# krea-ai/realtime-video

Hardware: AMD Instinct MI355X
Metric: frames/sec at 832x480, 4-step 14B T2V (per-step DiT latency in config) (higher is better)
Workload: dtype bf16

## Files before the change

### realtime_video_amd/csrc/vae_conv.hip

```cpp
#include "gemm_core.h"
#include "rtv_internal.h"

namespace rtv {

struct ConvParams {
  const uint16_t* in;
  const uint16_t* w;
  uint16_t* out;
  const uint16_t* bias;
  const uint16_t* residual;
  const uint16_t* zeros;
  int out_ld, res_ld;
  int T, H, W;
  int inH, inW;
  int Cin, Cout;
  int kt, kh, kw;
  int w_taps;
  int ups;
  int sy, st;
  int pad_h, pad_w;
  int limH, limW;
  int y_out0, y_in0;
  int in_rows;
  int gather;
// ... 513 lines not shown
    const int n = n0 + c * 8;
    u32x4 tv = *(const u32x4*)(img + conv_img_off<TN>(row, c, 0));
    if (y >= p.H || x >= p.W) continue;
    const size_t m = ((size_t)t * p.H + y) * p.W + x;
    if (p.residual) {
      const u32x4 rr = res_pre[ps];
#pragma unroll
      for (int i = 0; i < 4; ++i) {
        float a0, a1, r0, r1;
        unpack_f16x2(tv[i], a0, a1);
        unpack_f16x2(rr[i], r0, r1);
        tv[i] = pack_f16x2(a0 + r0, a1 + r1);
      }
    }
    *(u32x4*)(p.out + m * p.out_ld + n) = tv;
  }
}

namespace ch4 {
using namespace ch;
constexpr int THREADS4 = 256;
constexpr int HP = 10, WP = 5;
constexpr int A_ACC = 0, A_FRAG = 192, FRAG_SET = 28;
template <int ACC, int WF, int AF>
__device__ __forceinline__ void mfma_aaa() {
  asm volatile("v_mfma_f32_32x32x16_f16 a[%c0:%c1], a[%c2:%c3], a[%c4:%c5], a[%c0:%c1]" ::"n"(ACC), "n"(ACC + 15), "n"(WF), "n"(WF + 3),
               "n"(AF), "n"(AF + 3));
}
template <int DST, int OFF>
__device__ __forceinline__ void lds_read128_a(uint32_t lds_addr) {
  asm volatile("ds_read_b128 a[%c1:%c2], %0 offset:%3" ::"v"(lds_addr), "n"(DST), "n"(DST + 3), "n"(OFF));
}
template <int DST>
__device__ __forceinline__ void acc_zero() {
  asm volatile("v_accvgpr_write_b32 a[%c0], 0" ::"n"(DST));
}
template <int SRC>
__device__ __forceinline__ float acc_read() {
  float r;
  asm volatile("v_accvgpr_read_b32 %0, a[%c1]" : "=v"(r) : "n"(SRC));
  return r;
}
#define RTV_CH4_ACC \
  "a0", "a15", "a31", "a47", "a63", "a79", "a95", "a111", "a127", "a143", "a159", "a175", "a191", "a207", "a223", "a239", "a247"
}

template <int LAB>
__global__ __launch_bounds__(ch4::THREADS4, 1) void conv_halo4_kernel(ConvParams p, int tiles_x, int tiles_y) {
  using namespace ch4;
  extern __shared__ __attribute__((aligned(16))) char smem[];
  const int tid = threadIdx.x;
  const int lane = tid & 63;
  const int wave = __builtin_amdgcn_readfirstlane(tid >> 6);
  const int l31 = lane & 31, gl = lane >> 5;

  const int tiles_n = p.Cout / 96;
  const int id = xcd_remap(blockIdx.x, p.T * tiles_y * tiles_x * tiles_n);
  const int tn = id % tiles_n;
  int rest = id / tiles_n;
  const int tx = rest % tiles_x;
  rest /= tiles_x;
  const int ty = rest % tiles_y, t = rest / tiles_y;
  const int x0 = tx * TW, y0 = ty * TH, n0 = tn * 96;

  const int cpk = p.Cin / 32;
  const int G = p.kt * cpk;
  const int slice = p.inH * p.inW * p.Cin;
  const int taps = p.w_taps;

  uint32_t h_voff[HP], h_lds[HP];
#pragma unroll
  for (int i = 0; i < HP; ++i) {
    const int piece = min(wave * HP + i, HREAL - 1);
    h_lds[i] = piece * 1024;
    const int q = piece * 16 + (lane >> 2);
    const int hr = q / HPITCH, hc = q - hr * HPITCH;
    const int y = y0 - 1 + hr, x = x0 - 1 + hc;
    const int yi = p.y_out0 + y;
    const bool ok = q < HPIX && yi >= 0 && yi < p.limH && x >= 0 && x < p.limW;
    const int ys = p.ups ? (yi >> 1) - p.y_in0 : y, xs = p.ups ? x >> 1 : x;
    const int c = (lane & 3) ^ ((hc >> 2) & 3);
    h_voff[i] = ok ? (uint32_t)(((t * p.inH + ys) * p.inW + xs) * p.Cin + c * 8) * 2u : 0x80000000u;
  }
  uint32_t w_voff[WP], w_lds[WP];
#pragma unroll
  for (int i = 0; i < WP; ++i) {
    int piece = wave * WP + i;
    if (piece >= WREAL) piece -= 2;
    w_lds[i] = piece * 1024;
    const int dx = piece / 6, f = (piece % 6) * 16 + (lane >> 2);
    const int c = (lane & 3) ^ ((f >> 2) & 3);
    w_voff[i] = (uint32_t)(((n0 + f) * taps + dx) * p.Cin + c * 8) * 2u;
  }
  const __amdgpu_buffer_rsrc_t rsrcI = __builtin_amdgcn_make_buffer_rsrc((void*)p.in, 0, 0x80000000, 0x00020000);
  const __amdgpu_buffer_rsrc_t rsrcW = __builtin_amdgcn_make_buffer_rsrc((void*)p.w, 0, 0x7fffffff, 0x00020000);
  const uint32_t lds0 = (uint32_t)(uintptr_t)(RTV_LDS const char*)smem;
  auto issue_h = [&](uint32_t soff, uint32_t buf, auto ic) __attribute__((always_inline)) {
    constexpr int I = decltype(ic)::value;
    RTV_LDS void* dst = (RTV_LDS void*)(uintptr_t)(lds0 + buf * (uint32_t)HBYTES + h_lds[I]);
    __builtin_amdgcn_raw_ptr_buffer_load_lds(rsrcI, dst, 16, h_voff[I], soff, 0, 0);
  };
  auto issue_w = [&](uint32_t soff, auto slotc, auto ic) __attribute__((always_inline)) {
    constexpr int I = decltype(ic)::value, SLOT = decltype(slotc)::value;
    RTV_LDS void* dst = (RTV_LDS void*)(uintptr_t)(lds0 + (uint32_t)(2 * HBYTES + SLOT * WROW_BYTES) + w_lds[I]);
    __builtin_amdgcn_raw_ptr_buffer_load_lds(rsrcW, dst, 16, w_voff[I], soff, 0, 0);
  };
  auto h_soff = [&](int dt, int cb) __attribute__((always_inline)) { return (uint32_t)(dt * slice + cb * 32) * 2u; };
  auto w_soff = [&](int dt, int cb, int dy) __attribute__((always_inline)) {
    return (uint32_t)((dt * 9 + dy * 3) * p.Cin + cb * 32) * 2u;
  };

  uint32_t a_base[3][2], b_addr[3][2];
#pragma unroll
  for (int ks = 0; ks < 2; ++ks) {
#pragma unroll
    for (int dx = 0; dx < 3; ++dx) {
      const int hc = l31 + dx;
      a_base[dx][ks] = lds0 + (uint32_t)(((4 * wave) * HPITCH + hc) * 64 + (((2 * ks + gl) ^ ((hc >> 2) & 3)) << 4));
    }
#pragma unroll
    for (int dy = 0; dy < 3; ++dy)
      b_addr[dy][ks] = lds0 + (uint32_t)(2 * HBYTES + dy * WROW_BYTES + l31 * 64 + (((2 * ks + gl) ^ ((l31 >> 2) & 3)) << 4));
  }
  uint32_t a_cur[3][2], a_nxt[3][2];
  auto frag_read = [&](auto dyc, auto cic, auto setc, auto nc, const uint32_t (&aa)[3][2]) __attribute__((always_inline)) {
    constexpr int DY = decltype(dyc)::value, CI = decltype(cic)::value, SET = decltype(setc)::value, N = decltype(nc)::value;
    constexpr int dx = CI >> 1, ks = CI & 1;
    if constexpr (N < 3) lds_read128_a<A_FRAG + FRAG_SET * SET + 4 * N, dx * (96 * 64) + N * (32 * 64)>(b_addr[DY][ks]);
    else lds_read128_a<A_FRAG + FRAG_SET * SET + 12 + 4 * (N - 3), ((N - 3) + DY) * (HPITCH * 64)>(aa[dx][ks]);
  };

  asm volatile("" ::: RTV_CH4_ACC);
  sfor<0, 192>([&](auto ic) __attribute__((always_inline)) { acc_zero<A_ACC + decltype(ic)::value>(); });

  sfor<0, HP>([&](auto ic) __attribute__((always_inline)) { issue_h(h_soff(0, 0), 0u, ic); });
  sfor<0, WP>([&](auto ic) __attribute__((always_inline)) { issue_w(w_soff(0, 0, 0), IC<0>{}, ic); });
  sfor<0, WP>([&](auto ic) __attribute__((always_inline)) { issue_w(w_soff(0, 0, 1), IC<1>{}, ic); });
  asm volatile("s_waitcnt vmcnt(5)" ::: "memory");
  __builtin_amdgcn_s_barrier();
#pragma unroll
  for (int ks = 0; ks < 2; ++ks)
#pragma unroll
    for (int dx = 0; dx < 3; ++dx) a_cur[dx][ks] = a_base[dx][ks];
  sfor<0, 7>([&](auto nc) __attribute__((always_inline)) { frag_read(IC<0>{}, IC<0>{}, IC<0>{}, nc, a_cur); });

  int dt = 0, cb = 0;
  for (int g = 0; g < G; ++g) {
    const uint32_t nsel = (g & 1) ? 0u : (uint32_t)HBYTES;
    const bool more = g + 1 < G;
    const int cb1 = cb + 1 == cpk ? 0 : cb + 1, dt1 = cb + 1 == cpk ? dt + 1 : dt;
    uint32_t ws[3], hs;
    ws[0] = w_soff(dt, cb, 2);
    ws[1] = more ? w_soff(dt1, cb1, 0) : ws[0];
    ws[2] = more ? w_soff(dt1, cb1, 1) : ws[0];
    hs = more ? h_soff(dt1, cb1) : h_soff(dt, cb);
    const uint32_t nbuf = (uint32_t)((g + 1) & 1);
#pragma unroll
    for (int ks = 0; ks < 2; ++ks)
#pragma unroll
      for (int dx = 0; dx < 3; ++dx) a_nxt[dx][ks] = a_base[dx][ks] + nsel;
    sfor<0, 3>([&](auto dyc) __attribute__((always_inline)) {
      constexpr int DY = decltype(dyc)::value;
      sfor<0, 6>([&](auto cic) __attribute__((always_inline)) {
        constexpr int CI = decltype(cic)::value, SET = CI & 1;
        asm volatile("s_waitcnt lgkmcnt(0)");
        sfor<0, 12>([&](auto nc) __attribute__((always_inline)) {
          constexpr int n = decltype(nc)::value, mi = n / 3, ni = n % 3;
          mfma_aaa<A_ACC + (mi * 3 + ni) * 16, A_FRAG + FRAG_SET * SET + 4 * ni, A_FRAG + FRAG_SET * SET + 12 + 4 * mi>();
          __builtin_amdgcn_sched_barrier(0);
          if constexpr (CI < 5) {
            if constexpr (n < 7) frag_read(dyc, IC<CI + 1>{}, IC<SET ^ 1>{}, nc, a_cur);
            if constexpr (LAB != 1) {
              if constexpr (CI == 0 && n >= 7) issue_w(ws[DY], IC<(DY + 2) % 3>{}, IC<n - 7>{});
              if constexpr (DY == 0 && (CI == 1 || CI == 2) && n >= 7) issue_h(hs, nbuf, IC<(CI - 1) * 5 + n - 7>{});
            }
          } else {
            if constexpr (n == 2) {
              if constexpr (LAB == 1) asm volatile("s_waitcnt vmcnt(0)" ::: "memory");
              else if constexpr (DY == 2) asm volatile("s_waitcnt vmcnt(5)" ::: "memory");
              else asm volatile("s_waitcnt vmcnt(15)" ::: "memory");
              __builtin_amdgcn_s_barrier();
              __builtin_amdgcn_sched_barrier(0);
            }
            if constexpr (n >= 3 && n < 10) {
              if constexpr (DY < 2) frag_read(IC<DY + 1>{}, IC<0>{}, IC<SET ^ 1>{}, IC<n - 3>{}, a_cur);
              else frag_read(IC<0>{}, IC<0>{}, IC<SET ^ 1>{}, IC<n - 3>{}, a_nxt);
            }
          }
          __builtin_amdgcn_sched_barrier(0);
        });
      });
    });
#pragma unroll
    for (int ks = 0; ks < 2; ++ks)
#pragma unroll
      for (int dx = 0; dx < 3; ++dx) a_cur[dx][ks] = a_nxt[dx][ks];
    dt = dt1;
    cb = cb1;
  }
  asm volatile("s_waitcnt lgkmcnt(0)");
  asm volatile("s_waitcnt vmcnt(0)" ::: "memory");
  __builtin_amdgcn_s_barrier();
  asm volatile("s_nop 15\n\ts_nop 7");
  if constexpr (LAB == 2) {
    if (acc_read<0>() == 12345.678f) p.out[tid] = 1;
    return;
  }

  constexpr int TM = 4, TN = 3, CPR = TN * 4;
  u32x4 res_pre[TM * 32 * CPR / 64];
  if (p.residual) {
#pragma unroll
    for (int ps = 0; ps < TM * 32 * CPR / 64; ++ps) {
      const int q = ps * 64 + lane;
      const int row = q / CPR, c = q - row * CPR;
      const int y = y0 + 4 * wave + (row >> 5), x = x0 + (row & 31);
      res_pre[ps] = u32x4{0u, 0u, 0u, 0u};
      if (y < p.H && x < p.W) res_pre[ps] = *(const u32x4*)(p.residual + (((size_t)t * p.H + y) * p.W + x) * p.res_ld + n0 + c * 8);
    }
  }
  char* img = smem + wave * (TM * 32 * TN * 64);
  sfor<0, TM>([&](auto mic) __attribute__((always_inline)) {
    constexpr int mi = decltype(mic)::value;
    f32x16 accv[TN];
    sfor<0, TN * 16>([&](auto ic) __attribute__((always_inline)) {
      constexpr int i = decltype(ic)::value;
      accv[i >> 4][i & 15] = acc_read<A_ACC + mi * 48 + i>();
    });
    const int row = mi * 32 + l31;
    float yv[TN][4][4];
    float ssq = 0.f;
#pragma unroll
    for (int ni = 0; ni < TN; ++ni)
#pragma unroll
      for (int rq = 0; rq < 4; ++rq) {
        const int n = n0 + ni * 32 + rq * 8 + gl * 4;
        float v[4] = {accv[ni][rq * 4 + 0], accv[ni][rq * 4 + 1], accv[ni][rq * 4 + 2], accv[ni][rq * 4 + 3]};
        if (p.bias) {
          const u32x2 bb = *(const u32x2*)(p.bias + n);
          v[0] += f16_to_f32(bb[0] & 0xffff);
          v[1] += f16_to_f32(bb[0] >> 16);
          v[2] += f16_to_f32(bb[1] & 0xffff);
          v[3] += f16_to_f32(bb[1] >> 16);
        }
        u32x2 o;
        o[0] = pack_f16x2(v[0], v[1]);
        o[1] = pack_f16x2(v[2], v[3]);
        if (p.norm_gamma) {
          unpack_f16x2(o[0], yv[ni][rq][0], yv[ni][rq][1]);
          unpack_f16x2(o[1], yv[ni][rq][2], yv[ni][rq][3]);
#pragma unroll
          for (int i = 0; i < 4; ++i) ssq += yv[ni][rq][i] * yv[ni][rq][i];
        } else {
          *(u32x2*)(img + conv_img_off<TN>(row, ni * 4 + rq, gl)) = o;
        }
      }
    if (p.norm_gamma) {
      ssq += __shfl_xor(ssq, 32, 64);
      const float inv = sqrtf(96.f) / fmaxf(sqrtf(ssq), 1e-12f);
#pragma unroll
      for (int ni = 0; ni < TN; ++ni)
#pragma unroll
        for (int rq = 0; rq < 4; ++rq) {
          const u32x2 gg = *(const u32x2*)(p.norm_gamma + ni * 32 + rq * 8 + gl * 4);
          float g4[4];
          unpack_f16x2(gg[0], g4[0], g4[1]);
          unpack_f16x2(gg[1], g4[2], g4[3]);
          float z[4];
#pragma unroll
          for (int i = 0; i < 4; ++i) z[i] = silu(yv[ni][rq][i] * inv * g4[i]);
          u32x2 o;
          o[0] = pack_f16x2(z[0], z[1]);
          o[1] = pack_f16x2(z[2], z[3]);
          *(u32x2*)(img + conv_img_off<TN>(row, ni * 4 + rq, gl)) = o;
        }
    }
  });
  asm volatile("s_waitcnt lgkmcnt(0)" ::: "memory");
  __builtin_amdgcn_sched_barrier(0);
  constexpr int PASSES = TM * 32 * CPR / 64;
#pragma unroll
  for (int ps = 0; ps < PASSES; ++ps) {
    const int q = ps * 64 + lane;
    const int row = q / CPR, c = q - row * CPR;
    const int y = y0 + 4 * wave + (row >> 5), x = x0 + (row & 31);
    const int n = n0 + c * 8;
    u32x4 tv = *(const u32x4*)(img + conv_img_off<TN>(row, c, 0));
    if (y >= p.H || x >= p.W) continue;
    const size_t m = ((size_t)t * p.H + y) * p.W + x;
    if (p.residual) {
      const u32x4 rr = res_pre[ps];
#pragma unroll
      for (int i = 0; i < 4; ++i) {
        float a0, a1, r0, r1;
        unpack_f16x2(tv[i], a0, a1);
        unpack_f16x2(rr[i], r0, r1);
        tv[i] = pack_f16x2(a0 + r0, a1 + r1);
      }
    }
    *(u32x4*)(p.out + m * p.out_ld + n) = tv;
  }
}

__global__ __attribute__((amdgpu_flat_work_group_size(256, 256), amdgpu_waves_per_eu(1, 2))) void conv_halo4p_kernel(ConvParams p, int tiles_x,
                                                                                                                      int tiles_y) {
  using namespace ch4;
  constexpr int A_ACC = 8, A_FRAG = 200;
  extern __shared__ __attribute__((aligned(16))) char smem[];
  const int tid = threadIdx.x;
  const int lane = tid & 63;
  const int wave = __builtin_amdgcn_readfirstlane(tid >> 6);
  const int l31 = lane & 31, gl = lane >> 5;

  const int tiles_n = p.Cout / 96;
  const int total = p.T * tiles_y * tiles_x * tiles_n;
  const int stride = gridDim.x;
  const int cpk = p.Cin / 32;
  const int G = p.kt * cpk;
  const int slice = p.inH * p.inW * p.Cin;
  const int taps = p.w_taps;

  auto decode = [&](int vid, int& t, int& y0, int& x0, int& n0) __attribute__((always_inline)) {
    const int id = xcd_remap(vid, total);
    const int tn = id % tiles_n;
    int rest = id / tiles_n;
    const int tx = rest % tiles_x;
    rest /= tiles_x;
    const int ty = rest % tiles_y;
    t = rest / tiles_y;
    x0 = tx * TW;
    y0 = ty * TH;
    n0 = tn * 96;
  };
  uint32_t h_lds[HP], w_lds[WP];
#pragma unroll
  for (int i = 0; i < HP; ++i) h_lds[i] = min(wave * HP + i, HREAL - 1) * 1024;
#pragma unroll
  for (int i = 0; i < WP; ++i) w_lds[i] = (wave * WP + i >= WREAL ? wave * WP + i - 2 : wave * WP + i) * 1024;
  auto tile_voff = [&](int t, int y0, int x0, int n0, uint32_t (&hv)[HP], uint32_t (&wv)[WP]) __attribute__((always_inline)) {
    int lane_v = lane, wave_v = wave;
    asm volatile("" : "+v"(lane_v), "+s"(wave_v));
#pragma unroll
    for (int i = 0; i < HP; ++i) {
      const int piece = min(wave_v * HP + i, HREAL - 1);
      const int q = piece * 16 + (lane_v >> 2);
      const int hr = q / HPITCH, hc = q - hr * HPITCH;
      const int y = y0 - 1 + hr, x = x0 - 1 + hc;
      const int yi = p.y_out0 + y;
      const bool ok = q < HPIX && yi >= 0 && yi < p.limH && x >= 0 && x < p.limW;
      const int ys = p.ups ? (yi >> 1) - p.y_in0 : y, xs = p.ups ? x >> 1 : x;
      const int c = (lane_v & 3) ^ ((hc >> 2) & 3);
      hv[i] = ok ? (uint32_t)(((t * p.inH + ys) * p.inW + xs) * p.Cin + c * 8) * 2u : 0x80000000u;
    }
#pragma unroll
    for (int i = 0; i < WP; ++i) {
      int piece = wave_v * WP + i;
      if (piece >= WREAL) piece -= 2;
      const int dx = piece / 6, f = (piece % 6) * 16 + (lane_v >> 2);
      const int c = (lane_v & 3) ^ ((f >> 2) & 3);
      wv[i] = (uint32_t)(((n0 + f) * taps + dx) * p.Cin + c * 8) * 2u;
    }
  };
  const __amdgpu_buffer_rsrc_t rsrcI = __builtin_amdgcn_make_buffer_rsrc((void*)p.in, 0, 0x80000000, 0x00020000);
  const __amdgpu_buffer_rsrc_t rsrcW = __builtin_amdgcn_make_buffer_rsrc((void*)p.w, 0, 0x7fffffff, 0x00020000);
  const uint32_t lds0 = (uint32_t)(uintptr_t)(RTV_LDS const char*)smem;
  auto issue_h = [&](uint32_t soff, uint32_t buf, uint32_t voff, auto ic) __attribute__((always_inline)) {
    constexpr int I = decltype(ic)::value;
    RTV_LDS void* dst = (RTV_LDS void*)(uintptr_t)(lds0 + buf * (uint32_t)HBYTES + h_lds[I]);
    __builtin_amdgcn_raw_ptr_buffer_load_lds(rsrcI, dst, 16, voff, soff, 0, 0);
  };
  auto issue_w = [&](uint32_t soff, auto slotc, uint32_t voff, auto ic) __attribute__((always_inline)) {
    constexpr int I = decltype(ic)::value, SLOT = decltype(slotc)::value;
    RTV_LDS void* dst = (RTV_LDS void*)(uintptr_t)(lds0 + (uint32_t)(2 * HBYTES + SLOT * WROW_BYTES) + w_lds[I]);
    __builtin_amdgcn_raw_ptr_buffer_load_lds(rsrcW, dst, 16, voff, soff, 0, 0);
  };
  auto h_soff = [&](int dt, int cb) __attribute__((always_inline)) { return (uint32_t)(dt * slice + cb * 32) * 2u; };
  auto w_soff = [&](int dt, int cb, int dy) __attribute__((always_inline)) {
    return (uint32_t)((dt * 9 + dy * 3) * p.Cin + cb * 32) * 2u;
  };

  uint32_t a_base[3][2], b_addr[3][2];
  auto frag_addrs = [&]() __attribute__((always_inline)) {
    int lane_k = lane, wave_k = wave;
    asm volatile("" : "+v"(lane_k), "+s"(wave_k));
    const int l31k = lane_k & 31, glk = lane_k >> 5;
#pragma unroll
    for (int ks = 0; ks < 2; ++ks) {
#pragma unroll
      for (int dx = 0; dx < 3; ++dx) {
        const int hc = l31k + dx;
        a_base[dx][ks] = lds0 + (uint32_t)(((4 * wave_k) * HPITCH + hc) * 64 + (((2 * ks + glk) ^ ((hc >> 2) & 3)) << 4));
      }
#pragma unroll
      for (int dy = 0; dy < 3; ++dy)
        b_addr[dy][ks] = lds0 + (uint32_t)(2 * HBYTES + dy * WROW_BYTES + l31k * 64 + (((2 * ks + glk) ^ ((l31k >> 2) & 3)) << 4));
    }
  };
  frag_addrs();
  uint32_t a_cur[3][2], a_nxt[3][2];
  auto frag_read = [&](auto dyc, auto cic, auto setc, auto nc, const uint32_t (&aa)[3][2]) __attribute__((always_inline)) {
    constexpr int DY = decltype(dyc)::value, CI = decltype(cic)::value, SET = decltype(setc)::value, N = decltype(nc)::value;
    constexpr int dx = CI >> 1, ks = CI & 1;
    if constexpr (N < 3) lds_read128_a<A_FRAG + FRAG_SET * SET + 4 * N, dx * (96 * 64) + N * (32 * 64)>(b_addr[DY][ks]);
    else lds_read128_a<A_FRAG + FRAG_SET * SET + 12 + 4 * (N - 3), ((N - 3) + DY) * (HPITCH * 64)>(aa[dx][ks]);
  };

  asm volatile("" ::: RTV_CH4_ACC, "a255");
  sfor<0, 192>([&](auto ic) __attribute__((always_inline)) { acc_zero<A_ACC + decltype(ic)::value>(); });

  int vid = blockIdx.x;
  int ct, cy0, cx0, cn0;
  uint32_t hv_c[HP], wv_c[WP], hv_n[HP], wv_n[WP];
  decode(vid, ct, cy0, cx0, cn0);
  tile_voff(ct, cy0, cx0, cn0, hv_c, wv_c);

  sfor<0, HP>([&](auto ic) __attribute__((always_inline)) { issue_h(h_soff(0, 0), 0u, hv_c[decltype(ic)::value], ic); });
  sfor<0, WP>([&](auto ic) __attribute__((always_inline)) { issue_w(w_soff(0, 0, 0), IC<0>{}, wv_c[decltype(ic)::value], ic); });
  sfor<0, WP>([&](auto ic) __attribute__((always_inline)) { issue_w(w_soff(0, 0, 1), IC<1>{}, wv_c[decltype(ic)::value], ic); });
  asm volatile("s_waitcnt vmcnt(5)" ::: "memory");
  __builtin_amdgcn_s_barrier();
  uint32_t par = 0u;
#pragma unroll
  for (int ks = 0; ks < 2; ++ks)
#pragma unroll
    for (int dx = 0; dx < 3; ++dx) a_cur[dx][ks] = a_base[dx][ks];
  sfor<0, 7>([&](auto nc) __attribute__((always_inline)) { frag_read(IC<0>{}, IC<0>{}, IC<0>{}, nc, a_cur); });

  for (bool first_tile = true;; first_tile = false) {
    const bool has_next = vid + stride < total;
    if (!first_tile) {
      frag_addrs();
#pragma unroll
      for (int ks = 0; ks < 2; ++ks)
#pragma unroll
        for (int dx = 0; dx < 3; ++dx) a_cur[dx][ks] = a_base[dx][ks] + par * (uint32_t)HBYTES;
      tile_voff(ct, cy0, cx0, cn0, hv_c, wv_c);
    }
    {
      int nt = ct, ny0 = cy0, nx0 = cx0, nn0 = cn0;
      if (has_next) decode(vid + stride, nt, ny0, nx0, nn0);
      tile_voff(nt, ny0, nx0, nn0, hv_n, wv_n);
    }
    int dt = 0, cb = 0;
    for (int g = 0; g < G; ++g) {
      const bool last = g + 1 == G;
      const int cb1 = last ? 0 : (cb + 1 == cpk ? 0 : cb + 1), dt1 = last ? 0 : (cb + 1 == cpk ? dt + 1 : dt);
      uint32_t ws[3], hs;
      ws[0] = w_soff(dt, cb, 2);
      ws[1] = w_soff(dt1, cb1, 0);
      ws[2] = w_soff(dt1, cb1, 1);
      hs = h_soff(dt1, cb1);
      const uint32_t nbuf = par ^ 1u;
#pragma unroll
      for (int ks = 0; ks < 2; ++ks)
#pragma unroll
        for (int dx = 0; dx < 3; ++dx) a_nxt[dx][ks] = a_base[dx][ks] + nbuf * (uint32_t)HBYTES;
      sfor<0, 3>([&](auto dyc) __attribute__((always_inline)) {
        constexpr int DY = decltype(dyc)::value;
        sfor<0, 6>([&](auto cic) __attribute__((always_inline)) {
          constexpr int CI = decltype(cic)::value, SET = CI & 1;
          asm volatile("s_waitcnt lgkmcnt(0)");
          sfor<0, 12>([&](auto nc) __attribute__((always_inline)) {
            constexpr int n = decltype(nc)::value, mi = n / 3, ni = n % 3;
            mfma_aaa<A_ACC + (mi * 3 + ni) * 16, A_FRAG + FRAG_SET * SET + 4 * ni, A_FRAG + FRAG_SET * SET + 12 + 4 * mi>();
            __builtin_amdgcn_sched_barrier(0);
            if constexpr (CI < 5) {
              if constexpr (n < 7) frag_read(dyc, IC<CI + 1>{}, IC<SET ^ 1>{}, nc, a_cur);
              if constexpr (CI == 0 && n >= 7) {
                if constexpr (DY == 0) issue_w(ws[0], IC<2>{}, wv_c[n - 7], IC<n - 7>{});
                else issue_w(ws[DY], IC<DY - 1>{}, last ? wv_n[n - 7] : wv_c[n - 7], IC<n - 7>{});
              }
              if constexpr (DY == 0 && (CI == 1 || CI == 2) && n >= 7)
                issue_h(hs, nbuf, last ? hv_n[(CI - 1) * 5 + n - 7] : hv_c[(CI - 1) * 5 + n - 7], IC<(CI - 1) * 5 + n - 7>{});
            } else {
              if constexpr (n == 2) {
                if constexpr (DY == 2) {
                  asm volatile("s_waitcnt vmcnt(5)" ::: "memory");
                } else if constexpr (DY == 1) {
                  asm volatile("s_waitcnt vmcnt(15)" ::: "memory");
                } else {
                  if (g == 0) asm volatile("s_waitcnt vmcnt(0)" ::: "memory");
                  else asm volatile("s_waitcnt vmcnt(15)" ::: "memory");
                }
                __builtin_amdgcn_s_barrier();
                __builtin_amdgcn_sched_barrier(0);
              }
              if constexpr (n >= 3 && n < 10) {
                if constexpr (DY < 2) frag_read(IC<DY + 1>{}, IC<0>{}, IC<SET ^ 1>{}, IC<n - 3>{}, a_cur);
                else frag_read(IC<0>{}, IC<0>{}, IC<SET ^ 1>{}, IC<n - 3>{}, a_nxt);
              }
            }
            __builtin_amdgcn_sched_barrier(0);
          });
        });
      });
#pragma unroll
      for (int ks = 0; ks < 2; ++ks)
#pragma unroll
        for (int dx = 0; dx < 3; ++dx) a_cur[dx][ks] = a_nxt[dx][ks];
      par = nbuf;
      dt = dt1;
      cb = cb1;
    }

    asm volatile("s_nop 15\n\ts_nop 7");
    {
      constexpr int TN = 3, CPR = TN * 4, PPM = 32 * CPR / 64;
      int lane_e = lane, wave_e = wave;
      asm volatile("" : "+v"(lane_e), "+s"(wave_e));
      const int l31e = lane_e & 31, gle = lane_e >> 5;
      char* img = smem + LDS_BYTES + wave_e * (32 * TN * 64);
      u32x2 bias_pre[TN * 4];
      if (p.bias) {
#pragma unroll
        for (int j = 0; j < TN * 4; ++j) bias_pre[j] = *(const u32x2*)(p.bias + cn0 + (j >> 2) * 32 + (j & 3) * 8 + gle * 4);
      }
      u32x4 res_pre[PPM];
      auto res_load = [&](auto mic) __attribute__((always_inline)) {
        constexpr int mi = decltype(mic)::value;
#pragma unroll
        for (int ps = 0; ps < PPM; ++ps) {
          const int q = ps * 64 + lane_e;
          const int row = q / CPR, c = q - row * CPR;
          const int y = min(cy0 + 4 * wave_e + mi, p.H - 1), x = min(cx0 + row, p.W - 1);
          res_pre[ps] = *(const u32x4*)(p.residual + (((size_t)ct * p.H + y) * p.W + x) * p.res_ld + cn0 + c * 8);
        }
      };
      if (p.residual) res_load(IC<0>{});
      sfor<0, 4>([&](auto mic) __attribute__((always_inline)) {
        constexpr int mi = decltype(mic)::value;
        f32x16 accv[TN];
        sfor<0, TN * 16>([&](auto ic) __attribute__((always_inline)) {
          constexpr int i = decltype(ic)::value;
          accv[i >> 4][i & 15] = acc_read<A_ACC + mi * 48 + i>();
        });
        sfor<0, TN * 16>([&](auto ic) __attribute__((always_inline)) { acc_zero<A_ACC + mi * 48 + decltype(ic)::value>(); });
        const int row = l31e;
        u32x2 ypk[TN * 4];
        float ssq = 0.f;
#pragma unroll
        for (int ni = 0; ni < TN; ++ni)
#pragma unroll
          for (int rq = 0; rq < 4; ++rq) {
            float v[4] = {accv[ni][rq * 4 + 0], accv[ni][rq * 4 + 1], accv[ni][rq * 4 + 2], accv[ni][rq * 4 + 3]};
            if (p.bias) {
              const u32x2 bb = bias_pre[ni * 4 + rq];
              v[0] += f16_to_f32(bb[0] & 0xffff);
              v[1] += f16_to_f32(bb[0] >> 16);
              v[2] += f16_to_f32(bb[1] & 0xffff);
              v[3] += f16_to_f32(bb[1] >> 16);
            }
            u32x2 o;
            o[0] = pack_f16x2(v[0], v[1]);
            o[1] = pack_f16x2(v[2], v[3]);
            if (p.norm_gamma) {
              float y4[4];
              unpack_f16x2(o[0], y4[0], y4[1]);
              unpack_f16x2(o[1], y4[2], y4[3]);
#pragma unroll
              for (int i = 0; i < 4; ++i) ssq += y4[i] * y4[i];
              ypk[ni * 4 + rq] = o;
            } else {
              *(u32x2*)(img + conv_img_off<TN>(row, ni * 4 + rq, gle)) = o;
            }
          }
        if (p.norm_gamma) {
          ssq += __shfl_xor(ssq, 32, 64);
          const float inv = sqrtf(96.f) / fmaxf(sqrtf(ssq), 1e-12f);
#pragma unroll
          for (int ni = 0; ni < TN; ++ni)
#pragma unroll
            for (int rq = 0; rq < 4; ++rq) {
              const u32x2 gg = *(const u32x2*)(p.norm_gamma + ni * 32 + rq * 8 + gle * 4);
              float g4[4], y4[4];
              unpack_f16x2(gg[0], g4[0], g4[1]);
              unpack_f16x2(gg[1], g4[2], g4[3]);
              unpack_f16x2(ypk[ni * 4 + rq][0], y4[0], y4[1]);
              unpack_f16x2(ypk[ni * 4 + rq][1], y4[2], y4[3]);
              float z[4];
#pragma unroll
              for (int i = 0; i < 4; ++i) z[i] = silu(y4[i] * inv * g4[i]);
              u32x2 o;
              o[0] = pack_f16x2(z[0], z[1]);
              o[1] = pack_f16x2(z[2], z[3]);
              *(u32x2*)(img + conv_img_off<TN>(row, ni * 4 + rq, gle)) = o;
            }
        }
        asm volatile("s_waitcnt lgkmcnt(0)" ::: "memory");
        __builtin_amdgcn_sched_barrier(0);
#pragma unroll
        for (int ps = 0; ps < PPM; ++ps) {
          const int q = ps * 64 + lane_e;
          const int r = q / CPR, c = q - r * CPR;
          const int y = cy0 + 4 * wave_e + mi, x = cx0 + r;
          const int n = cn0 + c * 8;
          u32x4 tv = *(const u32x4*)(img + conv_img_off<TN>(r, c, 0));
          if (y >= p.H || x >= p.W) continue;
          const size_t m = ((size_t)ct * p.H + y) * p.W + x;
          if (p.residual) {
            const u32x4 rr = res_pre[ps];
#pragma unroll
            for (int i = 0; i < 4; ++i) {
              float a0, a1, r0, r1;
              unpack_f16x2(tv[i], a0, a1);
              unpack_f16x2(rr[i], r0, r1);
              tv[i] = pack_f16x2(a0 + r0, a1 + r1);
            }
          }
          *(u32x4*)(p.out + m * p.out_ld + n) = tv;
        }
        if constexpr (mi + 1 < 4) {
          if (p.residual) res_load(IC<mi + 1>{});
        }
      });
    }
    if (!has_next) break;
    vid += stride;
    decode(vid, ct, cy0, cx0, cn0);
  }
  asm volatile("s_waitcnt lgkmcnt(0)");
  asm volatile("s_waitcnt vmcnt(0)" ::: "memory");
}

static int launch_conv_halo(ConvParams p, hipStream_t stream, int form) {
  const int tiles_x = (p.W + ch::TW - 1) / ch::TW, tiles_y = (p.H + ch::TH - 1) / ch::TH;
  static LdsAttr lds_attr[5];
  const void* kern = form == 1 ? (const void*)conv_halo4_kernel<0> : form == 4 ? (const void*)conv_halo4p_kernel : (const void*)conv_halo_kernel;
#ifdef RTV_LAB
  if (form == 2) kern = (const void*)conv_halo4_kernel<1>;
  if (form == 3) kern = (const void*)conv_halo4_kernel<2>;
#endif
  const int lds = form == 4 ? ch::LDS_BYTES + 4 * 32 * 192 : ch::LDS_BYTES;
  if (int st = ensure_dynamic_lds(kern, lds, &lds_attr[form], "conv")) return st;
  ProfScope prof(PROF_CONV, stream, 2.0 * p.M * (double)p.Cout * 9 * p.kt * p.Cin);
  const dim3 grid(p.T * tiles_y * tiles_x * (p.Cout / 96));
  note_kernel(form == 4 ? DK_CONV_HALO4P : form == 0 ? DK_CONV_HALO : DK_CONV_HALO4);
  if (form == 4) {
    const int cus = device_num_cus() > 0 ? device_num_cus() : 256;
    const int nwg = (int)grid.x < cus ? (int)grid.x : cus / 8 * 8;
    hipLaunchKernelGGL(conv_halo4p_kernel, dim3(nwg), dim3(ch4::THREADS4), lds, stream, p, tiles_x, tiles_y);
    return check_launch("conv_halo");
  }
  if (form == 1) hipLaunchKernelGGL(conv_halo4_kernel<0>, grid, dim3(ch4::THREADS4), ch::LDS_BYTES, stream, p, tiles_x, tiles_y);
#ifdef RTV_LAB
  else if (form == 2) hipLaunchKernelGGL(conv_halo4_kernel<1>, grid, dim3(ch4::THREADS4), ch::LDS_BYTES, stream, p, tiles_x, tiles_y);
  else if (form == 3) hipLaunchKernelGGL(conv_halo4_kernel<2>, grid, dim3(ch4::THREADS4), ch::LDS_BYTES, stream, p, tiles_x, tiles_y);
#endif
  else hipLaunchKernelGGL(conv_halo_kernel, grid, dim3(ch::THREADS), ch::LDS_BYTES, stream, p, tiles_x, tiles_y);
  return check_launch("conv_halo");
}

template <int BM, int BN, int BK, int WM, int WN>
static int launch_conv_cfg(ConvParams p, hipStream_t stream) {
  typedef TileCfg<BM, BN, BK, WM, WN> Cfg;
  p.tiles_m = (p.M + BM - 1) / BM;
  p.tiles_n = (p.Cout + BN - 1) / BN;
  const int lds = 3 * Cfg::STAGE_BYTES;
  static_assert(Cfg::NW * Cfg::TM * 32 * Cfg::TN * 64 <= 3 * Cfg::STAGE_BYTES, "epilogue image must fit the stage buffers");
  auto kern = conv_igemm_kernel<BM, BN, BK, WM, WN>;
  static LdsAttr lds_attr;
  if (int st = ensure_dynamic_lds((const void*)kern, lds, &lds_attr, "conv")) return st;
  ProfScope prof(PROF_CONV, stream, 2.0 * p.M * (double)p.Cout * p.kt * p.kh * p.kw * p.Cin);
  note_kernel(DK_CONV_IGEMM);
  hipLaunchKernelGGL(kern, dim3(p.tiles_m * p.tiles_n), dim3(Cfg::NT), lds, stream, p);
  return check_launch("conv");
}

static std::atomic<int> g_conv_halo{1};

int launch_conv(const ConvParams& p, hipStream_t stream) {
  if (p.M <= 0) return 0;
  if (p.Cin % 32) return set_error(-1, "conv: Cin must be a multiple of 32 (pad channels)");
  if (p.Cout % 8) return set_error(-1, "conv: Cout must be a multiple of 8 (pad filters)");
  if (p.out_ld % 4 || (p.residual && p.res_ld % 4)) return set_error(-1, "conv: channel strides must be multiples of 4");
  if (p.n_split && (p.n_split % 4 || p.Cout != 2 * p.n_split)) return set_error(-1, "conv: bad n_split");
  const bool halo_common = g_conv_halo && !p.gather && p.kh == 3 && p.kw == 3 && p.sy == 1 && p.st == 1 && !p.n_split && p.pad_h == 1 &&
                           p.pad_w == 1 && p.Cin % 32 == 0 && p.Cin <= 384 && p.Cout % 96 == 0 && p.Cout <= 384 &&
                           !((p.out_ld | (p.residual ? p.res_ld : 0)) & 7) && !(((uintptr_t)p.out | (uintptr_t)p.residual) & 15) &&
                           (size_t)(p.T + 2) * p.inH * p.inW * p.Cin < 0x7fffffffull;
  const bool halo3 = halo_common && p.kt == 3 && !p.ups && p.y_out0 == 0 && p.y_in0 == 0 && p.in_rows == p.inH && p.limH == p.inH &&
                     p.limW == p.inW;
  const bool halo_up = halo_common && p.kt == 1 && p.ups && p.limW == p.W;
  const bool halo1 = halo_common && p.kt == 1 && !p.ups && p.w_taps == 27 && p.y_out0 == 0 && p.y_in0 == 0 && p.in_rows == p.inH &&
                     p.limH == p.inH && p.limW == p.inW;
  const bool halo = halo3 || halo_up || halo1;
  if (p.norm_gamma && !(halo && p.Cout == 96 && !p.residual && !((uintptr_t)p.norm_gamma & 7)))
    return set_error(-1, "conv: the fused RMS_norm + SiLU epilogue needs a halo-kernel layer with 96 filters and no residual");
  if (halo) {
    const int mode = g_conv_halo;
    int form = mode == 1 || mode == 6 ? 4 : mode == 2 ? 1 : mode == 3 ? 0 : mode - 2;
    if (form != 0 && (size_t)(p.T + 2) * p.inH * p.inW * p.Cin * 2 >= 0x80000000ull) form = 0;
    return launch_conv_halo(p, stream, form);
  }
  if (p.Cout % 96 == 0 && p.Cout % 128 != 0) return launch_conv_cfg<128, 96, 32, 2, 1>(p, stream);
  if (p.Cout <= 32) return launch_conv_cfg<128, 32, 32, 2, 1>(p, stream);
  return launch_conv_cfg<128, 128, 32, 2, 2>(p, stream);
}

}

using namespace rtv;

extern "C" int rtv_conv_set_halo(int on) {
#ifdef RTV_LAB
  g_conv_halo = on < 0 || on > 6 ? 1 : on;
#else
  g_conv_halo = on < 0 || (on > 3 && on != 6) ? 1 : on;
#endif
  return 0;
}

extern "C" int rtv_conv_cl_win(const void* in, const void* w, const void* bias, const void* residual, int res_ld,
                               void* out, int out_ld, int T, int H, int W, int Cin, int Cout, int kt, int kh, int kw,
                               int resample, int n_split, const void* zeros, int y_out0, int y_in0, int in_rows,
                               int img_rows, rtv_stream_t stream);

extern "C" int rtv_conv_cl(const void* in, const void* w, const void* bias, const void* residual, int res_ld,
                           void* out, int out_ld, int T, int H, int W, int Cin, int Cout, int kt, int kh, int kw,
                           int resample, int n_split, const void* zeros, rtv_stream_t stream) {
  return rtv_conv_cl_win(in, w, bias, residual, res_ld, out, out_ld, T, H, W, Cin, Cout, kt, kh, kw, resample, n_split,
                         zeros, 0, 0, -1, -1, stream);
}

static std::atomic<bool> g_conv_fuse_norm{true};
extern "C" int rtv_conv_set_fuse_norm(int on) {
  g_conv_fuse_norm = on != 0;
  return 0;
}

extern "C" int rtv_conv3_norm_silu_cl(const void* in, const void* w, const void* bias, const void* gamma, void* out, int out_ld,
                                      int T, int H, int W, int Cin, int Cout, int flags, const void* zeros, rtv_stream_t stream) {
  if (!in || !w || !out || !zeros || !gamma) return set_error(-1, "conv: null pointer");
  if (!g_conv_fuse_norm || !g_conv_halo || (flags & RTV_CONV_GATHER) || Cout != 96 || Cin % 32 || Cin > 384 || (out_ld & 7) ||
      ((uintptr_t)out & 15) || ((uintptr_t)gamma & 7) || (size_t)(T + 2) * H * W * Cin >= 0x7fffffffull)
    return 1;
  ConvParams p;
  p.in = (const uint16_t*)in;
  p.w = (const uint16_t*)w;
  p.out = (uint16_t*)out;
  p.bias = (const uint16_t*)bias;
  p.residual = nullptr;
  p.zeros = (const uint16_t*)zeros;
  p.out_ld = out_ld;
  p.res_ld = 0;
  p.T = T;
  p.H = H;
  p.W = W;
  p.inH = H;
  p.inW = W;
  p.sy = p.st = 1;
  p.pad_h = p.pad_w = 1;
  p.limH = H;
  p.limW = W;
  p.y_out0 = p.y_in0 = 0;
  p.in_rows = H;
  p.gather = 0;
  p.norm_gamma = (const uint16_t*)gamma;
  p.Cin = Cin;
  p.Cout = Cout;
  p.kt = p.kh = p.kw = 3;
  p.w_taps = 27;
  p.ups = 0;
  p.n_split = 0;
  p.M = T * H * W;
  p.tiles_m = p.tiles_n = 0;
  return launch_conv(p, (hipStream_t)stream);
}

int rtv::conv3_last_tap(const void* frame, const void* w3, const void* bias, const void* gamma, const void* residual, int res_ld,
                        void* out, int out_ld, int H, int W, int Cin, int Cout, int flags, const void* zeros, hipStream_t stream) {
  if (!frame || !w3 || !out || !zeros) return set_error(-1, "conv: null pointer");
  const int gather = (flags & RTV_CONV_GATHER) ? 1 : 0;
  if (gamma && (!g_conv_fuse_norm || !g_conv_halo || gather || Cout != 96 || Cin % 32 || Cin > 384 || (out_ld & 7) || residual ||
                ((uintptr_t)out & 15) || ((uintptr_t)gamma & 7)))
    return 1;
  ConvParams p;
  p.in = (const uint16_t*)frame;
  p.w = (const uint16_t*)w3 + (size_t)18 * Cin;
  p.out = (uint16_t*)out;
  p.bias = (const uint16_t*)bias;
  p.residual = (const uint16_t*)residual;
  p.zeros = (const uint16_t*)zeros;
  p.out_ld = out_ld;
  p.res_ld = res_ld;
  p.T = 1;
  p.H = H;
  p.W = W;
  p.inH = H;
  p.inW = W;
  p.sy = p.st = 1;
  p.pad_h = p.pad_w = 1;
  p.limH = H;
  p.limW = W;
  p.y_out0 = p.y_in0 = 0;
  p.in_rows = H;
  p.gather = gather;
  p.norm_gamma = (const uint16_t*)gamma;
  p.Cin = Cin;
  p.Cout = Cout;
  p.kt = 1;
  p.kh = p.kw = 3;
  p.w_taps = 27;
  p.ups = 0;
  p.n_split = 0;
  p.M = H * W;
  p.tiles_m = p.tiles_n = 0;
  return launch_conv(p, stream);
}

extern "C" int rtv_conv_cl_win(const void* in, const void* w, const void* bias, const void* residual, int res_ld,
                               void* out, int out_ld, int T, int H, int W, int Cin, int Cout, int kt, int kh, int kw,
                               int resample, int n_split, const void* zeros, int y_out0, int y_in0, int in_rows,
                               int img_rows, rtv_stream_t stream) {
  if (!in || !w || !out || !zeros) return set_error(-1, "conv: null pointer");
  const int gather = (resample & RTV_CONV_GATHER) ? 1 : 0;
  resample &= ~RTV_CONV_GATHER;
  if ((kt != 1 && kt != 3) || (kh != 1 && kh != 3) || kh != kw) return set_error(-1, "conv: kernel must be 1 or 3 per axis");
  if (resample < 0 || resample > 3) return set_error(-1, "conv: resample must be 0..3");
  const int ups = resample == RTV_CONV_UPSAMPLE2X;
  if (ups && ((W & 1) || (in_rows < 0 && (H & 1)))) return set_error(-1, "conv: upsampled output dims must be even");
  if (resample == RTV_CONV_DOWN2X && (kt != 1 || kh != 3)) return set_error(-1, "conv: the stride-2 downsample is a 1x3x3 conv");
  if (resample == RTV_CONV_TIME_DOWN2X && (kt != 3 || kh != 1)) return set_error(-1, "conv: the stride-2 time conv is 3x1x1");
  if (resample != RTV_CONV_NONE && resample != RTV_CONV_UPSAMPLE2X && n_split) return set_error(-1, "conv: n_split with a strided conv");
  ConvParams p;
  p.in = (const uint16_t*)in;
  p.w = (const uint16_t*)w;
  p.out = (uint16_t*)out;
  p.bias = (const uint16_t*)bias;
  p.residual = (const uint16_t*)residual;
  p.zeros = (const uint16_t*)zeros;
  p.out_ld = out_ld;
  p.res_ld = res_ld;
  p.T = T;
  p.H = H;
  p.W = W;
  p.inH = ups ? H / 2 : (resample == RTV_CONV_DOWN2X ? 2 * H : H);
  p.inW = ups ? W / 2 : (resample == RTV_CONV_DOWN2X ? 2 * W : W);
  p.sy = resample == RTV_CONV_DOWN2X ? 2 : 1;
  p.st = resample == RTV_CONV_TIME_DOWN2X ? 2 : 1;
  p.pad_h = resample == RTV_CONV_DOWN2X ? 0 : kh >> 1;
  p.pad_w = resample == RTV_CONV_DOWN2X ? 0 : kw >> 1;
  p.limH = ups ? H : p.inH;
  p.limW = ups ? W : p.inW;
  p.y_out0 = p.y_in0 = 0;
  p.in_rows = p.inH;
  if (in_rows >= 0) {
    if (!ups) return set_error(-1, "conv: row windows are for the upsampling stage transition");
    if (in_rows <= 0 || img_rows <= 0 || y_out0 < 0 || y_in0 < 0 || y_out0 + H > img_rows)
      return set_error(-1, "conv: bad row window");
    {
      const int lo_up = y_out0 > 0 ? y_out0 - (kh >> 1) : 0;
      const int hi_up = y_out0 + H - 1 + (kh >> 1) < img_rows ? y_out0 + H - 1 + (kh >> 1) : img_rows - 1;
      if ((lo_up >> 1) < y_in0 || (hi_up >> 1) >= y_in0 + in_rows)
        return set_error(-1, "conv: the row window's taps fall outside the supplied input rows");
    }
    p.y_out0 = y_out0;
    p.y_in0 = y_in0;
    p.in_rows = in_rows;
    p.inH = in_rows;
    p.limH = img_rows;
  }
  p.gather = gather;
  p.norm_gamma = nullptr;
  p.Cin = Cin;
  p.Cout = Cout;
  p.kt = kt;
  p.kh = kh;
  p.kw = kw;
  p.w_taps = kt * kh * kw;
  p.ups = ups ? 1 : 0;
  p.n_split = n_split;
  p.M = T * H * W;
  p.tiles_m = p.tiles_n = 0;
  return launch_conv(p, (hipStream_t)stream);
}
```

Baseline: 17.58.

## Split tail-round conv tiles into half-row units and skip dead rows

```diff
diff --git a/realtime_video_amd/csrc/vae_conv.hip b/realtime_video_amd/csrc/vae_conv.hip
--- a/realtime_video_amd/csrc/vae_conv.hip
+++ b/realtime_video_amd/csrc/vae_conv.hip
@@ -839,8 +839,8 @@
   }
 }
 
-__global__ __attribute__((amdgpu_flat_work_group_size(256, 256), amdgpu_waves_per_eu(1, 2))) void conv_halo4p_kernel(ConvParams p, int tiles_x,
-                                                                                                                      int tiles_y) {
+template <bool HALF>
+__device__ __forceinline__ void conv_halo4p_body(const ConvParams& p, int tiles_x, int tiles_y, int tail, int skip_dead) {
   using namespace ch4;
   constexpr int A_ACC = 8, A_FRAG = 200;
   extern __shared__ __attribute__((aligned(16))) char smem[];
@@ -869,6 +869,24 @@
     y0 = ty * TH;
     n0 = tn * 96;
   };
+  const int half_from = total - tail, vtotal = total + tail;
+  auto unit_of = [&](int v, int& t, int& y0, int& x0, int& n0, int& rb, int& mr) __attribute__((always_inline)) {
+    int u = v, half = 0;
+    mr = 4;
+    if (v >= half_from) {
+      const int h = v - half_from;
+      half = h >= tail ? 1 : 0;
+      u = v - half * tail;
+      mr = 2;
+    }
+    decode(u, t, y0, x0, n0);
+    if (HALF && skip_dead && mr == 4 && p.H - y0 <= TH / 2) mr = 2;
+    rb = half * (TH / 2) + mr * wave;
+  };
+  auto rows_of = [&](int y0, int rb, int mr) __attribute__((always_inline)) {
+    const int live = p.H - (y0 + rb);
+    return !skip_dead ? mr : live <= 0 ? 0 : HALF && live <= 2 ? 2 : mr;
+  };
   uint32_t h_lds[HP], w_lds[WP];
 #pragma unroll
   for (int i = 0; i < HP; ++i) h_lds[i] = min(wave * HP + i, HREAL - 1) * 1024;
@@ -917,23 +935,22 @@
   };
 
   uint32_t a_base[3][2], b_addr[3][2];
-  auto frag_addrs = [&]() __attribute__((always_inline)) {
-    int lane_k = lane, wave_k = wave;
-    asm volatile("" : "+v"(lane_k), "+s"(wave_k));
+  auto frag_addrs = [&](int rb) __attribute__((always_inline)) {
+    int lane_k = lane;
+    asm volatile("" : "+v"(lane_k));
     const int l31k = lane_k & 31, glk = lane_k >> 5;
 #pragma unroll
     for (int ks = 0; ks < 2; ++ks) {
 #pragma unroll
       for (int dx = 0; dx < 3; ++dx) {
         const int hc = l31k + dx;
-        a_base[dx][ks] = lds0 + (uint32_t)(((4 * wave_k) * HPITCH + hc) * 64 + (((2 * ks + glk) ^ ((hc >> 2) & 3)) << 4));
+        a_base[dx][ks] = lds0 + (uint32_t)((rb * HPITCH + hc) * 64 + (((2 * ks + glk) ^ ((hc >> 2) & 3)) << 4));
       }
 #pragma unroll
       for (int dy = 0; dy < 3; ++dy)
         b_addr[dy][ks] = lds0 + (uint32_t)(2 * HBYTES + dy * WROW_BYTES + l31k * 64 + (((2 * ks + glk) ^ ((l31k >> 2) & 3)) << 4));
     }
   };
-  frag_addrs();
   uint32_t a_cur[3][2], a_nxt[3][2];
   auto frag_read = [&](auto dyc, auto cic, auto setc, auto nc, const uint32_t (&aa)[3][2]) __attribute__((always_inline)) {
     constexpr int DY = decltype(dyc)::value, CI = decltype(cic)::value, SET = decltype(setc)::value, N = decltype(nc)::value;
@@ -946,10 +963,11 @@
   sfor<0, 192>([&](auto ic) __attribute__((always_inline)) { acc_zero<A_ACC + decltype(ic)::value>(); });
 
   int vid = blockIdx.x;
-  int ct, cy0, cx0, cn0;
+  int ct, cy0, cx0, cn0, crb, cmr;
   uint32_t hv_c[HP], wv_c[WP], hv_n[HP], wv_n[WP];
-  decode(vid, ct, cy0, cx0, cn0);
+  unit_of(vid, ct, cy0, cx0, cn0, crb, cmr);
   tile_voff(ct, cy0, cx0, cn0, hv_c, wv_c);
+  frag_addrs(crb);
 
   sfor<0, HP>([&](auto ic) __attribute__((always_inline)) { issue_h(h_soff(0, 0), 0u, hv_c[decltype(ic)::value], ic); });
   sfor<0, WP>([&](auto ic) __attribute__((always_inline)) { issue_w(w_soff(0, 0, 0), IC<0>{}, wv_c[decltype(ic)::value], ic); });
@@ -963,21 +981,12 @@
     for (int dx = 0; dx < 3; ++dx) a_cur[dx][ks] = a_base[dx][ks];
   sfor<0, 7>([&](auto nc) __attribute__((always_inline)) { frag_read(IC<0>{}, IC<0>{}, IC<0>{}, nc, a_cur); });
 
-  for (bool first_tile = true;; first_tile = false) {
-    const bool has_next = vid + stride < total;
-    if (!first_tile) {
-      frag_addrs();
-#pragma unroll
-      for (int ks = 0; ks < 2; ++ks)
-#pragma unroll
-        for (int dx = 0; dx < 3; ++dx) a_cur[dx][ks] = a_base[dx][ks] + par * (uint32_t)HBYTES;
-      tile_voff(ct, cy0, cx0, cn0, hv_c, wv_c);
-    }
-    {
-      int nt = ct, ny0 = cy0, nx0 = cx0, nn0 = cn0;
-      if (has_next) decode(vid + stride, nt, ny0, nx0, nn0);
-      tile_voff(nt, ny0, nx0, nn0, hv_n, wv_n);
-    }
+  bool has_next;
+  int nrb;
+  int rows = 4;
+  auto unit_body = [&](auto mrc) __attribute__((always_inline)) {
+    constexpr int MR = decltype(mrc)::value;
+    const bool full = !HALF || rows == 4;
     int dt = 0, cb = 0;
     for (int g = 0; g < G; ++g) {
       const bool last = g + 1 == G;
@@ -988,21 +997,24 @@
       ws[2] = w_soff(dt1, cb1, 1);
       hs = h_soff(dt1, cb1);
       const uint32_t nbuf = par ^ 1u;
+      const uint32_t nrow = nbuf * (uint32_t)HBYTES + (last ? (uint32_t)((nrb - crb) * (HPITCH * 64)) : 0u);
 #pragma unroll
       for (int ks = 0; ks < 2; ++ks)
 #pragma unroll
-        for (int dx = 0; dx < 3; ++dx) a_nxt[dx][ks] = a_base[dx][ks] + nbuf * (uint32_t)HBYTES;
+        for (int dx = 0; dx < 3; ++dx) a_nxt[dx][ks] = a_base[dx][ks] + nrow;
       sfor<0, 3>([&](auto dyc) __attribute__((always_inline)) {
         constexpr int DY = decltype(dyc)::value;
         sfor<0, 6>([&](auto cic) __attribute__((always_inline)) {
           constexpr int CI = decltype(cic)::value, SET = CI & 1;
           asm volatile("s_waitcnt lgkmcnt(0)");
-          sfor<0, 12>([&](auto nc) __attribute__((always_inline)) {
-            constexpr int n = decltype(nc)::value, mi = n / 3, ni = n % 3;
-            mfma_aaa<A_ACC + (mi * 3 + ni) * 16, A_FRAG + FRAG_SET * SET + 4 * ni, A_FRAG + FRAG_SET * SET + 12 + 4 * mi>();
-            __builtin_amdgcn_sched_barrier(0);
+          auto slot = [&](auto nc, auto mfc, auto nrc) __attribute__((always_inline)) {
+            constexpr int n = decltype(nc)::value, mi = n / 3, ni = n % 3, NR = decltype(nrc)::value;
+            if constexpr (decltype(mfc)::value) {
+              mfma_aaa<A_ACC + (mi * 3 + ni) * 16, A_FRAG + FRAG_SET * SET + 4 * ni, A_FRAG + FRAG_SET * SET + 12 + 4 * mi>();
+              __builtin_amdgcn_sched_barrier(0);
+            }
             if constexpr (CI < 5) {
-              if constexpr (n < 7) frag_read(dyc, IC<CI + 1>{}, IC<SET ^ 1>{}, nc, a_cur);
+              if constexpr (n < NR) frag_read(dyc, IC<CI + 1>{}, IC<SET ^ 1>{}, nc, a_cur);
               if constexpr (CI == 0 && n >= 7) {
                 if constexpr (DY == 0) issue_w(ws[0], IC<2>{}, wv_c[n - 7], IC<n - 7>{});
                 else issue_w(ws[DY], IC<DY - 1>{}, last ? wv_n[n - 7] : wv_c[n - 7], IC<n - 7>{});
@@ -1023,12 +1035,22 @@
                 __builtin_amdgcn_sched_barrier(0);
               }
               if constexpr (n >= 3 && n < 10) {
-                if constexpr (DY < 2) frag_read(IC<DY + 1>{}, IC<0>{}, IC<SET ^ 1>{}, IC<n - 3>{}, a_cur);
-                else frag_read(IC<0>{}, IC<0>{}, IC<SET ^ 1>{}, IC<n - 3>{}, a_nxt);
+                if constexpr (DY < 2) {
+                  if constexpr (n - 3 < NR) frag_read(IC<DY + 1>{}, IC<0>{}, IC<SET ^ 1>{}, IC<n - 3>{}, a_cur);
+                } else {
+                  frag_read(IC<0>{}, IC<0>{}, IC<SET ^ 1>{}, IC<n - 3>{}, a_nxt);
+                }
               }
             }
             __builtin_amdgcn_sched_barrier(0);
-          });
+          };
+          if constexpr (MR == 0) {
+            sfor<0, 12>([&](auto nc) __attribute__((always_inline)) { slot(nc, IC<0>{}, IC<0>{}); });
+          } else {
+            sfor<0, 6>([&](auto nc) __attribute__((always_inline)) { slot(nc, IC<1>{}, IC<7>{}); });
+            if (full) sfor<6, 12>([&](auto nc) __attribute__((always_inline)) { slot(nc, IC<1>{}, IC<7>{}); });
+            else sfor<6, 12>([&](auto nc) __attribute__((always_inline)) { slot(nc, IC<0>{}, IC<5>{}); });
+          }
         });
       });
 #pragma unroll
@@ -1040,8 +1062,8 @@
       cb = cb1;
     }
 
-    asm volatile("s_nop 15\n\ts_nop 7");
-    {
+    if constexpr (MR > 0) {
+      asm volatile("s_nop 15\n\ts_nop 7");
       constexpr int TN = 3, CPR = TN * 4, PPM = 32 * CPR / 64;
       int lane_e = lane, wave_e = wave;
       asm volatile("" : "+v"(lane_e), "+s"(wave_e));
@@ -1059,13 +1081,14 @@
         for (int ps = 0; ps < PPM; ++ps) {
           const int q = ps * 64 + lane_e;
           const int row = q / CPR, c = q - row * CPR;
-          const int y = min(cy0 + 4 * wave_e + mi, p.H - 1), x = min(cx0 + row, p.W - 1);
+          const int y = min(cy0 + crb + mi, p.H - 1), x = min(cx0 + row, p.W - 1);
           res_pre[ps] = *(const u32x4*)(p.residual + (((size_t)ct * p.H + y) * p.W + x) * p.res_ld + cn0 + c * 8);
         }
       };
       if (p.residual) res_load(IC<0>{});
-      sfor<0, 4>([&](auto mic) __attribute__((always_inline)) {
+      sfor<0, MR>([&](auto mic) __attribute__((always_inline)) {
         constexpr int mi = decltype(mic)::value;
+        if (mi >= rows) return;
         f32x16 accv[TN];
         sfor<0, TN * 16>([&](auto ic) __attribute__((always_inline)) {
           constexpr int i = decltype(ic)::value;
@@ -1129,7 +1152,7 @@
         for (int ps = 0; ps < PPM; ++ps) {
           const int q = ps * 64 + lane_e;
           const int r = q / CPR, c = q - r * CPR;
-          const int y = cy0 + 4 * wave_e + mi, x = cx0 + r;
+          const int y = cy0 + crb + mi, x = cx0 + r;
           const int n = cn0 + c * 8;
           u32x4 tv = *(const u32x4*)(img + conv_img_off<TN>(r, c, 0));
           if (y >= p.H || x >= p.W) continue;
@@ -1146,20 +1169,51 @@
           }
           *(u32x4*)(p.out + m * p.out_ld + n) = tv;
         }
-        if constexpr (mi + 1 < 4) {
-          if (p.residual) res_load(IC<mi + 1>{});
+        if constexpr (mi + 1 < MR) {
+          if (p.residual && mi + 1 < rows) res_load(IC<mi + 1>{});
         }
       });
     }
+  };
+
+  for (bool first_unit = true;; first_unit = false) {
+    has_next = vid + stride < vtotal;
+    if (!first_unit) {
+      frag_addrs(crb);
+#pragma unroll
+      for (int ks = 0; ks < 2; ++ks)
+#pragma unroll
+        for (int dx = 0; dx < 3; ++dx) a_cur[dx][ks] = a_base[dx][ks] + par * (uint32_t)HBYTES;
+      tile_voff(ct, cy0, cx0, cn0, hv_c, wv_c);
+    }
+    {
+      int nt = ct, ny0 = cy0, nx0 = cx0, nn0 = cn0, nmr = cmr;
+      nrb = crb;
+      if (has_next) unit_of(vid + stride, nt, ny0, nx0, nn0, nrb, nmr);
+      tile_voff(nt, ny0, nx0, nn0, hv_n, wv_n);
+    }
+    rows = rows_of(cy0, crb, cmr);
+    if (rows) unit_body(IC<4>{});
+    else unit_body(IC<0>{});
     if (!has_next) break;
     vid += stride;
-    decode(vid, ct, cy0, cx0, cn0);
+    unit_of(vid, ct, cy0, cx0, cn0, crb, cmr);
   }
   asm volatile("s_waitcnt lgkmcnt(0)");
   asm volatile("s_waitcnt vmcnt(0)" ::: "memory");
 }
 
-static int launch_conv_halo(ConvParams p, hipStream_t stream, int form) {
+__global__ __attribute__((amdgpu_flat_work_group_size(256, 256), amdgpu_waves_per_eu(1, 2))) void conv_halo4p_kernel(ConvParams p, int tiles_x,
+                                                                                                                      int tiles_y, int skip_dead) {
+  conv_halo4p_body<false>(p, tiles_x, tiles_y, 0, skip_dead);
+}
+__global__ __attribute__((amdgpu_flat_work_group_size(256, 256), amdgpu_waves_per_eu(1, 2))) void conv_halo4h_kernel(ConvParams p, int tiles_x,
+                                                                                                                      int tiles_y, int tail,
+                                                                                                                      int skip_dead) {
+  conv_halo4p_body<true>(p, tiles_x, tiles_y, tail, skip_dead);
+}
+
+static int launch_conv_halo(ConvParams p, hipStream_t stream, int form, int tail_mode = 3) {
   const int tiles_x = (p.W + ch::TW - 1) / ch::TW, tiles_y = (p.H + ch::TH - 1) / ch::TH;
   static LdsAttr lds_attr[5];
   const void* kern = form == 1 ? (const void*)conv_halo4_kernel<0> : form == 4 ? (const void*)conv_halo4p_kernel : (const void*)conv_halo_kernel;
@@ -1175,7 +1229,16 @@
   if (form == 4) {
     const int cus = device_num_cus() > 0 ? device_num_cus() : 256;
     const int nwg = (int)grid.x < cus ? (int)grid.x : cus / 8 * 8;
-    hipLaunchKernelGGL(conv_halo4p_kernel, dim3(nwg), dim3(ch4::THREADS4), lds, stream, p, tiles_x, tiles_y);
+    const int r = (int)grid.x % nwg, rounds = ((int)grid.x + nwg - 1) / nwg, hrem = p.H % ch::TH;
+    const int tail = (tail_mode & 1) && (int)grid.x > nwg && r && 2 * r <= nwg ? r : 0;
+    const int skip_dead = (tail_mode >> 1) & 1;
+    if (rounds <= 8 && (tail || (skip_dead && hrem > 0 && hrem <= ch::TH / 2))) {
+      static LdsAttr lds_attr_h;
+      if (int st = ensure_dynamic_lds((const void*)conv_halo4h_kernel, lds, &lds_attr_h, "conv")) return st;
+      hipLaunchKernelGGL(conv_halo4h_kernel, dim3(nwg), dim3(ch4::THREADS4), lds, stream, p, tiles_x, tiles_y, tail, skip_dead);
+    } else {
+      hipLaunchKernelGGL(conv_halo4p_kernel, dim3(nwg), dim3(ch4::THREADS4), lds, stream, p, tiles_x, tiles_y, skip_dead);
+    }
     return check_launch("conv_halo");
   }
   if (form == 1) hipLaunchKernelGGL(conv_halo4_kernel<0>, grid, dim3(ch4::THREADS4), ch::LDS_BYTES, stream, p, tiles_x, tiles_y);
@@ -1225,9 +1288,9 @@
     return set_error(-1, "conv: the fused RMS_norm + SiLU epilogue needs a halo-kernel layer with 96 filters and no residual");
   if (halo) {
     const int mode = g_conv_halo;
-    int form = mode == 1 || mode == 6 ? 4 : mode == 2 ? 1 : mode == 3 ? 0 : mode - 2;
+    int form = mode == 1 || mode >= 6 ? 4 : mode == 2 ? 1 : mode == 3 ? 0 : mode - 2;
     if (form != 0 && (size_t)(p.T + 2) * p.inH * p.inW * p.Cin * 2 >= 0x80000000ull) form = 0;
-    return launch_conv_halo(p, stream, form);
+    return launch_conv_halo(p, stream, form, mode >= 7 ? mode - 7 : 3);
   }
   if (p.Cout % 96 == 0 && p.Cout % 128 != 0) return launch_conv_cfg<128, 96, 32, 2, 1>(p, stream);
   if (p.Cout <= 32) return launch_conv_cfg<128, 32, 32, 2, 1>(p, stream);
@@ -1240,9 +1303,9 @@
 
 extern "C" int rtv_conv_set_halo(int on) {
 #ifdef RTV_LAB
-  g_conv_halo = on < 0 || on > 6 ? 1 : on;
+  g_conv_halo = on < 0 || on > 9 ? 1 : on;
 #else
-  g_conv_halo = on < 0 || (on > 3 && on != 6) ? 1 : on;
+  g_conv_halo = on < 0 || (on > 3 && on < 6) || on > 9 ? 1 : on;
 #endif
   return 0;
 }
```

Result: no change. 17.51 (-0.4%).
